# joshuacwnewton/swiftwatcher

Hardware: AMD Instinct MI355X
Metric: frames/sec (segment+classify) on 1080p ROI batches (higher is better)
Workload: dtype f64 (image_filtering), f32 (CNN)

## Files before the change

### include/swk.h

```cpp
#ifndef SWK_H
#define SWK_H

#include <stdint.h>

#ifdef __cplusplus
extern "C" {
#endif

#define SWK_ABI_VERSION 2

enum {
    SWK_OK = 0,
    SWK_ERR_ARG = -1,
    SWK_ERR_HIP = -2,
    SWK_ERR_NOGPU = -3,
    SWK_ERR_CAPACITY = -4,
    SWK_ERR_NOMEM = -5,
    SWK_ERR_STALE = -6
};

enum { SWK_MEM_HOST = 0, SWK_MEM_DEVICE = 1 };

enum { SWK_ORDER_RASTER = 0, SWK_ORDER_BLOCK2X2 = 1 };

// ... 102 lines not shown
                           const swk_segment *segs, const int32_t *nseg, int32_t seg_cap, int32_t min_h, int32_t min_w,
                           const float mean[3], const float std_[3], int32_t pad, int32_t channels_last, int32_t first,
                           int32_t net_cap, float *net, int32_t *seg_frame, int32_t *total, int32_t *skipped);
int32_t swk_segment_inputs_last(swk_ctx *ctx, int32_t min_h, int32_t min_w, const float mean[3], const float std_[3],
                                int32_t pad, int32_t channels_last, int32_t first, int32_t net_cap, float *net,
                                int32_t *seg_frame, int32_t *total, int32_t *skipped);

int32_t swk_nhwc_bias_relu_place(void *stream, const float *src, int32_t n, int32_t sh, int32_t sw, int32_t c, int32_t crop_y,
                                 int32_t crop_x, int32_t h, int32_t w, const float *bias, float *dst, int32_t dH, int32_t dW,
                                 int32_t dC, int32_t off_y, int32_t off_x, int32_t c_off);
int32_t swk_nhwc_maxpool3s2(void *stream, const float *src, int32_t n, int32_t h, int32_t w, int32_t c, float *dst);
int32_t swk_nhwc_head2_relu_mean(void *stream, const float *x, int32_t n, int32_t px, int32_t c, const float *w, const float *bias,
                                 const float *ring, float n_pos, float *out);
int32_t swk_nhwc_conv7x7s2_bias_relu(void *stream, const float *src, int32_t n, int32_t side, int32_t lo, int32_t m, const float *weight,
                                     const float *bias, int32_t cout, float *dst);
int32_t swk_nhwc_conv1x1_bias_relu_place(void *stream, const float *src, int32_t n, int32_t sh, int32_t sw, int32_t cin, int32_t crop_y,
                                         int32_t crop_x, int32_t h, int32_t w, const float *weight, const float *bias, int32_t cout,
                                         float *dst, int32_t dH, int32_t dW, int32_t dC, int32_t off_y, int32_t off_x, int32_t c_off);

int32_t swk_nhwc_maxpool3s2_conv1x1_bias_relu_place(void *stream, const float *src, int32_t n, int32_t t, int32_t cin, const float *weight,
                                                    const float *bias, int32_t cout, float *dst, int32_t dH, int32_t dW, int32_t dC,
                                                    int32_t off_y, int32_t off_x, const float *ring, int32_t live_lo, int32_t live_n);


int32_t swk_nhwc_conv3x3_bias_relu_place(void *stream, const float *src, int32_t n, int32_t t, int32_t cin, const float *weight_t,
                                         const float *bias, int32_t cout, float *dst, int32_t dH, int32_t dW, int32_t dC, int32_t off_y,
                                         int32_t off_x, int32_t c_off);

int32_t swk_winograd_f2x2_3x3_weights(const float *weight, int32_t cout, int32_t cin, float *out);
int32_t swk_nhwc_conv3x3_winograd_bias_relu_place(void *stream, const float *src, int32_t n, int32_t t, int32_t cin, const float *weight_w,
                                                  const float *bias, int32_t cout, float *dst, int32_t dH, int32_t dW, int32_t dC,
                                                  int32_t off_y, int32_t off_x, int32_t c_off);

int32_t swk_track_costs(const double *prev_c, const double *prev_hist0, const uint8_t *prev_has_hist,
                        const double *curr_c, int32_t n_prev, int32_t n_curr, double *cost);
int32_t swk_lsap(const double *cost, int32_t n_rows, int32_t n_cols, int32_t *col4row);

int32_t swk_median_blur_u8(const uint8_t *src, int32_t H, int32_t W, int32_t channels, int32_t ksize, uint8_t *dst);
int32_t swk_otsu_threshold_u8(const uint8_t *src, int64_t count, uint8_t *dst, int32_t *thresh);
int32_t swk_canny_u8(const uint8_t *src, int32_t H, int32_t W, int32_t low, int32_t high, uint8_t *dst);
int32_t swk_dilate_up_u8(const uint8_t *src, int32_t H, int32_t W, int32_t N, uint8_t *dst);
int32_t swk_roi_mask(const uint8_t *frame, int32_t H, int32_t W, int64_t row_stride, const int32_t corners[4],
                     int32_t crop_region[4], uint8_t *mask, int64_t mask_capacity);


#ifdef __cplusplus
}
#endif
#endif
```

### swiftwatcher_amd/_lib.py

```python
import ctypes
import os
import threading

import numpy as np

_HERE = os.path.dirname(os.path.abspath(__file__))
LIB_PATH = os.environ.get("SWK_LIB", os.path.join(_HERE, "libswk.so"))

ABI_VERSION = 2
MEM_HOST, MEM_DEVICE = 0, 1
ERR_STALE = -6
STAGES = ("gray", "rpca", "bilateral", "thresh", "opened", "labels")
ORDER_RASTER, ORDER_BLOCK2X2 = 0, 1
GRAY_Q14, GRAY_Q15 = 0, 1
K_GRAY, K_IALM_STATS, K_IALM_PASS, K_IALM_SMALL, K_FILTER, K_CCL, K_PROPS, K_COPY = range(8)
KERNEL_FAMILIES = ["gray", "ialm_stats", "ialm_pass", "ialm_small", "filter", "ccl", "props", "copy"]

c_u8p = ctypes.POINTER(ctypes.c_uint8)
c_f64p = ctypes.POINTER(ctypes.c_double)
c_i32p = ctypes.POINTER(ctypes.c_int32)


class SwkError(RuntimeError):
    pass
# ... 52 lines not shown
    "swk_batch_run": (ctypes.c_int32, [ctypes.c_void_p, ctypes.POINTER(Input), ctypes.POINTER(Params), ctypes.POINTER(Output)]),
    "swk_batch_run_groups": (ctypes.c_int32, [ctypes.c_void_p, ctypes.POINTER(Input), ctypes.c_int32, ctypes.POINTER(Params), ctypes.POINTER(Output)]),
    "swk_bgr2gray": (ctypes.c_int32, [ctypes.c_void_p, ctypes.c_void_p, ctypes.c_int32, ctypes.c_int32, ctypes.c_int32, ctypes.c_int32, ctypes.c_void_p]),
    "swk_ialm": (ctypes.c_int32, [ctypes.c_void_p, ctypes.c_void_p, ctypes.c_int32, ctypes.c_int32, ctypes.c_double, ctypes.c_double, ctypes.c_int32, ctypes.c_void_p, ctypes.c_void_p, ctypes.c_void_p]),
    "swk_rpca_epilogue": (ctypes.c_int32, [ctypes.c_void_p, ctypes.c_void_p, ctypes.c_int64, ctypes.c_void_p]),
    "swk_bilateral_u8": (ctypes.c_int32, [ctypes.c_void_p, ctypes.c_void_p, ctypes.c_int32, ctypes.c_int32, ctypes.c_int32, ctypes.c_int32, ctypes.c_double, ctypes.c_double, ctypes.c_int32, ctypes.c_void_p]),
    "swk_thresh_tozero_u8": (ctypes.c_int32, [ctypes.c_void_p, ctypes.c_void_p, ctypes.c_int64, ctypes.c_int32, ctypes.c_void_p]),
    "swk_grey_open3x3_u8": (ctypes.c_int32, [ctypes.c_void_p, ctypes.c_void_p, ctypes.c_int32, ctypes.c_int32, ctypes.c_int32, ctypes.c_void_p]),
    "swk_grey_open_u8": (ctypes.c_int32, [ctypes.c_void_p, ctypes.c_void_p] + [ctypes.c_int32] * 5 + [ctypes.c_void_p]),
    "swk_resize_linear_u8": (ctypes.c_int32, [ctypes.c_void_p, ctypes.c_void_p] + [ctypes.c_int32] * 6 + [ctypes.c_void_p]),
    "swk_ccl_u8": (ctypes.c_int32, [ctypes.c_void_p, ctypes.c_void_p, ctypes.c_int32, ctypes.c_int32, ctypes.c_int32, ctypes.c_int32, ctypes.c_int32, ctypes.c_void_p, ctypes.c_void_p]),
    "swk_regionprops_u8": (ctypes.c_int32, [ctypes.c_void_p, ctypes.c_void_p, ctypes.c_int32, ctypes.c_int32, ctypes.c_int32, ctypes.c_int32, ctypes.c_void_p, ctypes.c_void_p]),
    "swk_classifier_input": (ctypes.c_int32, [ctypes.c_void_p, ctypes.c_void_p, ctypes.c_int64, ctypes.c_void_p, ctypes.c_void_p, ctypes.c_int32, ctypes.c_void_p, ctypes.c_void_p, ctypes.c_void_p, ctypes.c_void_p, ctypes.c_int32]),
    "swk_set_sparse_speculation": (ctypes.c_int32, [ctypes.c_void_p, ctypes.c_double]),
    "swk_set_integer_start": (ctypes.c_int32, [ctypes.c_void_p, ctypes.c_int32]),
    "swk_last_integer_start_windows": (ctypes.c_int32, [ctypes.c_void_p, ctypes.c_void_p]),
    "swk_last_eig_sweeps": (ctypes.c_int32, [ctypes.c_void_p, ctypes.c_void_p]),
    "swk_set_norm_speculation": (ctypes.c_int32, [ctypes.c_void_p, ctypes.c_double]),
    "swk_set_norm_guard": (ctypes.c_int32, [ctypes.c_void_p, ctypes.c_double]),
    "swk_prof_guard_windows": (ctypes.c_int32, [ctypes.c_void_p, ctypes.c_void_p]),
    "swk_last_stopping_norms": (ctypes.c_int32, [ctypes.c_void_p, ctypes.c_void_p, ctypes.c_void_p, ctypes.c_int32]),
    "swk_set_start_refine": (ctypes.c_int32, [ctypes.c_void_p, ctypes.c_double]),
    "swk_prof_refined_windows": (ctypes.c_int32, [ctypes.c_void_p, ctypes.c_void_p, ctypes.c_void_p]),
    "swk_prof_pass_bytes_per_element": (ctypes.c_int32, [ctypes.c_void_p, ctypes.c_void_p]),
    "swk_prof_redo_batches": (ctypes.c_int32, [ctypes.c_void_p, ctypes.c_void_p]),
    "swk_prof_redo_windows": (ctypes.c_int32, [ctypes.c_void_p, ctypes.c_void_p]),
    "swk_nhwc_bias_relu_place": (ctypes.c_int32, [ctypes.c_void_p, ctypes.c_void_p] + [ctypes.c_int32] * 8 + [ctypes.c_void_p, ctypes.c_void_p] + [ctypes.c_int32] * 6),
    "swk_set_cnn_tuning": (ctypes.c_int32, [ctypes.c_int32, ctypes.c_int32]),
    "swk_nhwc_conv7x7s2_bias_relu": (ctypes.c_int32, [ctypes.c_void_p, ctypes.c_void_p, ctypes.c_int32, ctypes.c_int32, ctypes.c_int32, ctypes.c_int32, ctypes.c_void_p, ctypes.c_void_p, ctypes.c_int32, ctypes.c_void_p]),
    "swk_nhwc_conv1x1_bias_relu_place": (ctypes.c_int32, [ctypes.c_void_p, ctypes.c_void_p] + [ctypes.c_int32] * 8 + [ctypes.c_void_p, ctypes.c_void_p, ctypes.c_int32, ctypes.c_void_p] + [ctypes.c_int32] * 6),
    "swk_nhwc_conv3x3_bias_relu_place": (ctypes.c_int32, [ctypes.c_void_p, ctypes.c_void_p, ctypes.c_int32, ctypes.c_int32, ctypes.c_int32, ctypes.c_void_p, ctypes.c_void_p, ctypes.c_int32, ctypes.c_void_p] + [ctypes.c_int32] * 6),
    "swk_nhwc_conv3x3_winograd_bias_relu_place": (ctypes.c_int32, [ctypes.c_void_p, ctypes.c_void_p, ctypes.c_int32, ctypes.c_int32, ctypes.c_int32, ctypes.c_void_p, ctypes.c_void_p, ctypes.c_int32, ctypes.c_void_p] + [ctypes.c_int32] * 6),
    "swk_winograd_f2x2_3x3_weights": (ctypes.c_int32, [ctypes.c_void_p, ctypes.c_int32, ctypes.c_int32, ctypes.c_void_p]),
    "swk_nhwc_maxpool3s2_conv1x1_bias_relu_place": (ctypes.c_int32, [ctypes.c_void_p, ctypes.c_void_p, ctypes.c_int32, ctypes.c_int32, ctypes.c_int32, ctypes.c_void_p, ctypes.c_void_p, ctypes.c_int32, ctypes.c_void_p] + [ctypes.c_int32] * 5 + [ctypes.c_void_p, ctypes.c_int32, ctypes.c_int32]),
    "swk_nhwc_maxpool3s2": (ctypes.c_int32, [ctypes.c_void_p, ctypes.c_void_p, ctypes.c_int32, ctypes.c_int32, ctypes.c_int32, ctypes.c_int32, ctypes.c_void_p]),
    "swk_nhwc_head2_relu_mean": (ctypes.c_int32, [ctypes.c_void_p, ctypes.c_void_p, ctypes.c_int32, ctypes.c_int32, ctypes.c_int32, ctypes.c_void_p,
                                                  ctypes.c_void_p, ctypes.c_void_p, ctypes.c_float, ctypes.c_void_p]),
    "swk_segment_inputs": (ctypes.c_int32, [ctypes.c_void_p, ctypes.c_void_p, ctypes.c_int32, ctypes.c_int32, ctypes.c_void_p, ctypes.c_void_p, ctypes.c_int32, ctypes.c_int32, ctypes.c_int32, ctypes.c_void_p, ctypes.c_void_p, ctypes.c_int32, ctypes.c_int32, ctypes.c_int32, ctypes.c_int32, ctypes.c_void_p, ctypes.c_void_p, ctypes.c_void_p, ctypes.c_void_p]),
    "swk_segment_inputs_last": (ctypes.c_int32, [ctypes.c_void_p, ctypes.c_int32, ctypes.c_int32, ctypes.c_void_p, ctypes.c_void_p, ctypes.c_int32, ctypes.c_int32, ctypes.c_int32, ctypes.c_int32, ctypes.c_void_p, ctypes.c_void_p, ctypes.c_void_p, ctypes.c_void_p]),
    "swk_device_alloc": (ctypes.c_int32, [ctypes.c_void_p, ctypes.c_int64, ctypes.POINTER(ctypes.c_void_p)]),
    "swk_device_free": (ctypes.c_int32, [ctypes.c_void_p, ctypes.c_void_p]),
    "swk_device_read": (ctypes.c_int32, [ctypes.c_void_p, ctypes.c_void_p, ctypes.c_void_p, ctypes.c_int64]),
    "swk_classifier_input_window": (ctypes.c_int32, [ctypes.c_void_p, ctypes.c_void_p, ctypes.c_int64, ctypes.c_void_p, ctypes.c_void_p, ctypes.c_int32, ctypes.c_void_p, ctypes.c_void_p, ctypes.c_int32, ctypes.c_int32, ctypes.c_void_p, ctypes.c_void_p, ctypes.c_int32]),
    "swk_track_costs": (ctypes.c_int32, [ctypes.c_void_p, ctypes.c_void_p, ctypes.c_void_p, ctypes.c_void_p, ctypes.c_int32, ctypes.c_int32, ctypes.c_void_p]),
    "swk_lsap": (ctypes.c_int32, [ctypes.c_void_p, ctypes.c_int32, ctypes.c_int32, ctypes.c_void_p]),
    "swk_median_blur_u8": (ctypes.c_int32, [ctypes.c_void_p, ctypes.c_int32, ctypes.c_int32, ctypes.c_int32, ctypes.c_int32, ctypes.c_void_p]),
    "swk_otsu_threshold_u8": (ctypes.c_int32, [ctypes.c_void_p, ctypes.c_int64, ctypes.c_void_p, ctypes.c_void_p]),
    "swk_canny_u8": (ctypes.c_int32, [ctypes.c_void_p, ctypes.c_int32, ctypes.c_int32, ctypes.c_int32, ctypes.c_int32, ctypes.c_void_p]),
    "swk_dilate_up_u8": (ctypes.c_int32, [ctypes.c_void_p, ctypes.c_int32, ctypes.c_int32, ctypes.c_int32, ctypes.c_void_p]),
    "swk_roi_mask": (ctypes.c_int32, [ctypes.c_void_p, ctypes.c_int32, ctypes.c_int32, ctypes.c_int64, ctypes.c_void_p, ctypes.c_void_p, ctypes.c_void_p, ctypes.c_int64]),
    "swk_pinned_alloc": (ctypes.c_int32, [ctypes.c_int32, ctypes.c_int64, ctypes.POINTER(ctypes.c_void_p)]),
    "swk_pinned_free": (ctypes.c_int32, [ctypes.c_void_p]),
    "swk_cut_boxes": (ctypes.c_int32, [ctypes.c_void_p, ctypes.c_int32, ctypes.c_int64, ctypes.c_int32, ctypes.c_int32, ctypes.c_void_p, ctypes.c_void_p, ctypes.c_void_p, ctypes.c_void_p]),
    "swk_stage_frames": (ctypes.c_int32, [ctypes.c_void_p, ctypes.c_int32, ctypes.c_int64, ctypes.c_int32, ctypes.c_int32, ctypes.c_int64, ctypes.c_int64, ctypes.c_void_p, ctypes.c_int32]),
    "swk_prof_enable": (ctypes.c_int32, [ctypes.c_void_p, ctypes.c_int32]),
    "swk_prof_reset": (ctypes.c_int32, [ctypes.c_void_p]),
    "swk_prof_get": (ctypes.c_int32, [ctypes.c_void_p, ctypes.c_int32, ctypes.POINTER(ctypes.c_double), ctypes.POINTER(ctypes.c_int64)]),
    "swk_prof_window_iters": (ctypes.c_int32, [ctypes.c_void_p, ctypes.POINTER(ctypes.c_int64)]),
    "swk_set_ialm_variant": (ctypes.c_int32, [ctypes.c_void_p, ctypes.c_int32]),
    "swk_set_pass_tuning": (ctypes.c_int32, [ctypes.c_void_p, ctypes.c_int32]),
    "swk_set_eig_method": (ctypes.c_int32, [ctypes.c_void_p, ctypes.c_int32]),
}
EXPORTS = sorted(_SIGS)


def _preload_torch_hip_runtime():
# ... 630 lines not shown
```

### swiftwatcher_amd/csrc/build.py

```python
import os
import subprocess
import sys

HERE = os.path.dirname(os.path.abspath(__file__))
PKG = os.path.dirname(HERE)
ROOT = os.path.dirname(PKG)
LIB = os.path.join(PKG, "libswk.so")
SOURCES = ["swk_api.hip", "ialm.hip", "ialm_mfma.hip", "ialm_mstate.hip", "ialm_small.hip", "ialm_refine.hip", "ialm_gram8.hip", "groups.hip", "filters.hip", "ccl.hip", "classify_input.hip", "cnn_aux.hip", "cnn_conv1.hip", "cnn_conv1x1.hip", "cnn_expand_bf16.hip", "cnn_conv3x3.hip", "cnn_wino3x3.hip", "cnn_poolsq.hip", "tracker.cpp", "roi_mask.cpp", "host_stage.cpp"]
HEADERS = ["swk_internal.h", "ialm_small_dev.h", os.path.join(ROOT, "include", "swk.h"), os.path.join(ROOT, "include", "swk_debug.h")]
FLAGS = ["--offload-arch=gfx950", "-O3", "-std=c++17", "-fPIC", "-ffp-contract=off",
         "-fvisibility=hidden", "-Wall", "-Wno-unused-function", "-I", os.path.join(ROOT, "include"), "-I", HERE]


def _stale(out, deps):
    if not os.path.exists(out):
        return True
    t = os.path.getmtime(out)
    return any(os.path.getmtime(d) > t for d in deps)


def build(force=False, verbose=False):
    hipcc = os.environ.get("HIPCC", "/opt/rocm/bin/hipcc")
    objdir = os.path.join(HERE, "build")
    os.makedirs(objdir, exist_ok=True)
    hdrs = [h if os.path.isabs(h) else os.path.join(HERE, h) for h in HEADERS]
    objs = []
    procs = []
    for src in SOURCES:
        sp = os.path.join(HERE, src)
        obj = os.path.join(objdir, src + ".o")
        objs.append(obj)
        if force or _stale(obj, [sp] + hdrs + [os.path.abspath(__file__)]):
            cmd = [hipcc] + FLAGS + ["-c", sp, "-o", obj]
            if verbose:
                print(" ".join(cmd))
            procs.append((src, subprocess.Popen(cmd)))
    for src, p in procs:
        if p.wait() != 0:
            raise RuntimeError("hipcc failed on " + src)
    if force or procs or _stale(LIB, objs):
        cmd = [hipcc, "--offload-arch=gfx950", "-shared", "-fPIC", "-pthread", "-o", LIB] + objs
# ... 9 lines not shown
```

### swiftwatcher_amd/segment_classification.py

```python
import ctypes
import os
import threading

import numpy as np
import torch
from torch import nn

IMAGENET_MEAN = (0.485, 0.456, 0.406)
IMAGENET_STD = (0.229, 0.224, 0.225)
RESIZE = 24
PAD = (224 - 24) // 2


class Fire(nn.Module):

    def __init__(self, inplanes, squeeze_planes, expand1x1_planes, expand3x3_planes):
        super().__init__()
        self.squeeze = nn.Conv2d(inplanes, squeeze_planes, kernel_size=1)
        self.squeeze_activation = nn.ReLU(inplace=True)
        self.expand1x1 = nn.Conv2d(squeeze_planes, expand1x1_planes, kernel_size=1)
        self.expand1x1_activation = nn.ReLU(inplace=True)
        self.expand3x3 = nn.Conv2d(squeeze_planes, expand3x3_planes, kernel_size=3, padding=1)
        self.expand3x3_activation = nn.ReLU(inplace=True)

# ... 74 lines not shown
                lo, hi = a, b
            else:
                out_size = maps[i + 1].shape[-1] if i + 1 < len(feats) else x.shape[-1]
                a, b = _affected(lo, hi, 3, 2, 0, out_size)
                n0, n1 = 2 * a, 2 * b + 2
                assert n0 >= 0 and n1 <= size - 1
                tile = in_map[:, :, n0:n1 + 1, n0:n1 + 1].contiguous()
                self.plan.append(("pool", layer, tile, lo - n0, hi - lo + 1, None, None))
                lo, hi, size = a, b, out_size
        self.final = (lo, hi, size)
        self.final_bg = x[:, :, lo:hi + 1, lo:hi + 1].contiguous()
        ring = head.clone()
        ring[:, :, lo:hi + 1, lo:hi + 1] = 0
        self.ring_sum = ring.sum(dim=(2, 3))
        self.n_pos = float(size * size)
        self.sq_bg = []
        with torch.no_grad():
            for kind, layer, tile, off, n, pad, crop in self.plan:
                if kind != "fire":
                    self.sq_bg.append(None)
                    continue
                sq = layer.squeeze_activation(layer.squeeze(tile))
                if pad[0] or pad[1]:
                    sq = torch.nn.functional.pad(sq, (pad[0], pad[1], pad[0], pad[1]))
                self.sq_bg.append(sq.contiguous())
        self._cap = 0
        self._buf = None
        self.memory_format = torch.channels_last if dev.type == "cuda" else torch.contiguous_format
        if self.memory_format == torch.channels_last:
            model.to(memory_format=torch.channels_last)
        self.own_kernels = os.environ.get("SWK_OWN_CNN_KERNELS", "1") == "1"
        self._head = None
        self.winograd = True
        self.fuse_pool = os.environ.get("SWK_FUSE_POOL", "1") == "1"
        self._w1 = None
        self._wt3 = {}
        self._ww3 = {}

    def macs_per_segment(self):
        m = self.model
        c1 = m.features[0]
        side = (self.IN_HI - self.IN_LO + 1 - 7) // 2 + 1
        executed = useful = side * side * c1.out_channels * c1.in_channels * 49
        last_n = None
        on_gpu = self.ring_sum.is_cuda and self.memory_format == torch.channels_last and self.own_kernels
        for kind, layer, tile, off, n, pad, crop in self.plan:
            if kind != "fire":
                continue
            t = tile.shape[2] + pad[0] + pad[1]
            sq, e1, e3 = layer.squeeze, layer.expand1x1, layer.expand3x3
            executed += n * n * sq.out_channels * sq.in_channels
            e1_side = n if on_gpu else t
            executed += e1_side * e1_side * e1.out_channels * e1.in_channels
            wino = on_gpu and self.winograd and e3.out_channels == 4 * e3.in_channels and e3.in_channels in (16, 32, 48, 64)
            if wino:
                tiles = ((t - 2 + 1) // 2) ** 2
                executed += tiles * 16 * e3.out_channels * e3.in_channels
            else:
                executed += (t - 2) ** 2 * e3.out_channels * e3.in_channels * 9
            useful += n * n * sq.out_channels * sq.in_channels
            useful += crop[1] ** 2 * (e1.out_channels * e1.in_channels + e3.out_channels * e3.in_channels * 9)
            last_n = crop[1]
        head = m.classifier[1]
        executed += last_n * last_n * head.out_channels * head.in_channels
        useful += last_n * last_n * head.out_channels * head.in_channels
        return int(executed), int(useful)

    def _buffers(self, batch):
        if batch <= self._cap:
            return self._buf
        bufs = []
        for (kind, layer, tile, off, n, pad, crop), sq in zip(self.plan, self.sq_bg):
            if kind == "fire":
                bufs.append(sq.expand(batch, -1, -1, -1).contiguous(memory_format=self.memory_format))
            else:
                bufs.append(tile.expand(batch, -1, -1, -1).contiguous(memory_format=self.memory_format))
        live = []
        for j, (kind, layer, tile, off, n, pad, crop) in enumerate(self.plan):
            nxt = self.plan[j + 1][0] if j + 1 < len(self.plan) else "head"
            if kind == "fire" and nxt != "pool":
                if nxt == "fire":
                    _, _, ntile, noff, nn, _, _ = self.plan[j + 1]
                    bg = ntile[:, :, noff:noff + nn, noff:noff + nn]
                else:
                    bg = self.final_bg
                assert bg.shape[2] == crop[1] and bg.shape[1] == layer.expand1x1.out_channels + layer.expand3x3.out_channels
                live.append(bg.expand(batch, -1, -1, -1).contiguous(memory_format=self.memory_format))
            else:
                live.append(None)
        self._buf, self._cap = (bufs, live), batch
        self.version = getattr(self, "version", 0) + 1
        return self._buf

    def _gpu_path(self, tiles):
        return tiles.is_cuda and self.memory_format == torch.channels_last and all(
            kind != "fire" or not (pad[0] or pad[1]) for kind, _, _, _, _, pad, _ in self.plan)

    def reserve(self, batch):
        self._buffers(batch)
        if self.ring_sum.is_cuda:
            self._aux_buffers(batch)

    @torch.no_grad()
    def __call__(self, tiles, row0=0):
        if self._gpu_path(tiles):
            with torch.cuda.device(tiles.device):
                return self._forward_hip_glue(tiles, row0)
        if row0:
            raise ValueError("row0 is a feature of the GPU path")
        m = self.model
        conv2d = torch.nn.functional.conv2d
        k = tiles.shape[0]
        bufs, live = self._buffers(k)
        x = torch.relu(m.features[0](tiles.contiguous(memory_format=self.memory_format)))
        a, b = self.pool1_slice
        x = m.features[2](x[:, :, a:b, a:b])
        for j, (kind, layer, tile, off, n, pad, crop) in enumerate(self.plan):
            if kind == "pool":
                x = layer(bufs[j][:k])
                continue
            sq = bufs[j][:k]
            o = off + pad[0]
            torch.clamp_min(layer.squeeze(x), 0, out=sq[:, :, o:o + n, o:o + n])
            e3 = conv2d(sq, layer.expand3x3.weight, layer.expand3x3.bias)
            e1 = conv2d(sq, layer.expand1x1.weight, layer.expand1x1.bias)
            c, cn = crop
            c1 = layer.expand1x1.out_channels
            if live[j] is not None:
                dest = live[j][:k]
            else:
                _, _, _, poff, pn, _, _ = self.plan[j + 1]
                assert pn == cn
                dest = bufs[j + 1][:k, :, poff:poff + pn, poff:poff + pn]
            cp = c + pad[0]
# ... 7 lines not shown
        from . import _lib
        lib = _lib.load()
        stream = ctypes.c_void_p(torch.cuda.current_stream(tiles.device).cuda_stream)
        m = self.model
        conv2d = torch.nn.functional.conv2d
        k = tiles.shape[0]
        bufs, live = self._buffers(row0 + k)
        rows = slice(row0, row0 + k)
        cl = torch.channels_last

        def nhwc(t):
            return t if t.is_contiguous(memory_format=cl) else t.contiguous(memory_format=cl)

        def place(e, bias, dest, crop, size, off, c_off):
            e = nhwc(e)
            rc = lib.swk_nhwc_bias_relu_place(stream, e.data_ptr(), k, e.shape[2], e.shape[3], e.shape[1], crop, crop, size, size,
                                              bias.data_ptr(), dest.data_ptr(), dest.shape[2], dest.shape[3], dest.shape[1],
                                              off, off, c_off)
            if rc:
                raise RuntimeError("swk_nhwc_bias_relu_place failed (%d)" % rc)

        def conv1x1(src, crop, size, conv, dest, off, c_off):
            src = nhwc(src)
            wgt = conv.weight.reshape(conv.out_channels, conv.in_channels)
            rc = lib.swk_nhwc_conv1x1_bias_relu_place(stream, src.data_ptr(), k, src.shape[2], src.shape[3], src.shape[1], crop, crop,
                                                      size, size, wgt.data_ptr(), conv.bias.data_ptr(), conv.out_channels,
                                                      dest.data_ptr(), dest.shape[2], dest.shape[3], dest.shape[1], off, off, c_off)
            if rc:
                raise RuntimeError("swk_nhwc_conv1x1_bias_relu_place failed (%d)" % rc)

        def conv3x3(src, j, conv, dest, off, c_off):
            src = nhwc(src)
            cin, cout = conv.in_channels, conv.out_channels
            if self.winograd and cout == 4 * cin and cin in (16, 32, 48, 64) and k * src.shape[2] * src.shape[2] * cin * 4 < (1 << 32):
                ww = self._ww3.get(j)
                if ww is None:
                    w = conv.weight.detach().to("cpu", torch.float32).contiguous()
                    out = torch.empty(16 * cin * cout, dtype=torch.float32)
                    if lib.swk_winograd_f2x2_3x3_weights(w.data_ptr(), cout, cin, out.data_ptr()):
                        raise RuntimeError("swk_winograd_f2x2_3x3_weights failed")
                    ww = self._ww3[j] = out.to(src.device)
                rc = lib.swk_nhwc_conv3x3_winograd_bias_relu_place(stream, src.data_ptr(), k, src.shape[2], cin, ww.data_ptr(),
                                                                   conv.bias.data_ptr(), cout, dest.data_ptr(), dest.shape[2],
                                                                   dest.shape[3], dest.shape[1], off, off, c_off)
                if rc:
                    raise RuntimeError("swk_nhwc_conv3x3_winograd_bias_relu_place failed (%d)" % rc)
                return
            wt = self._wt3.get(j)
            if wt is None:
                wt = self._wt3[j] = conv.weight.detach().permute(2, 3, 1, 0).contiguous(memory_format=torch.contiguous_format)
            assert src.shape[2] == src.shape[3]
            rc = lib.swk_nhwc_conv3x3_bias_relu_place(stream, src.data_ptr(), k, src.shape[2], src.shape[1], wt.data_ptr(),
                                                      conv.bias.data_ptr(), conv.out_channels, dest.data_ptr(), dest.shape[2],
                                                      dest.shape[3], dest.shape[1], off, off, c_off)
            if rc:
                raise RuntimeError("swk_nhwc_conv3x3_bias_relu_place failed (%d)" % rc)

        def pool(src, dst):
            rc = lib.swk_nhwc_maxpool3s2(stream, src.data_ptr(), k, src.shape[2], src.shape[3], src.shape[1], dst.data_ptr())
            if rc:
                raise RuntimeError("swk_nhwc_maxpool3s2 failed (%d)" % rc)

        def pool_squeeze(src, conv, dest, off, ring=None, live=(0, 0)):
            wgt = conv.weight.reshape(conv.out_channels, conv.in_channels)
            rc = lib.swk_nhwc_maxpool3s2_conv1x1_bias_relu_place(stream, src.data_ptr(), k, src.shape[2], src.shape[1], wgt.data_ptr(),
                                                                 conv.bias.data_ptr(), conv.out_channels, dest.data_ptr(), dest.shape[2],
                                                                 dest.shape[3], dest.shape[1], off, off,
                                                                 None if ring is None else ring.data_ptr(), live[0], live[1])
            if rc:
                raise RuntimeError("swk_nhwc_maxpool3s2_conv1x1_bias_relu_place failed (%d)" % rc)

        aux = self._aux_buffers(row0 + k)
        conv1 = m.features[0]
        a, b = self.pool1_slice
        c1buf = aux["conv1"][rows]
        side = tiles.shape[2]
        if self.own_kernels and conv1.out_channels == 96 and side % 2 == 0 and 2 * (b - 1) + 8 <= side:
            if self._w1 is None:
                self._w1 = conv1.weight.detach().contiguous(memory_format=torch.contiguous_format).clone()
            xin = nhwc(tiles)
            rc = lib.swk_nhwc_conv7x7s2_bias_relu(stream, xin.data_ptr(), k, side, a, b - a, self._w1.data_ptr(), conv1.bias.data_ptr(),
                                                  conv1.out_channels, c1buf.data_ptr())
            if rc:
                raise RuntimeError("swk_nhwc_conv7x7s2_bias_relu failed (%d)" % rc)
        else:
            e = conv2d(nhwc(tiles), conv1.weight, None, stride=conv1.stride)
            place(e, conv1.bias, c1buf, a, b - a, 0, 0)
        fuse = self.fuse_pool and self.own_kernels
        to_pool = c1buf
        pool_ring, pool_live = None, (0, 0)
        x = aux["pool_in"][rows]
        if not fuse:
            pool(c1buf, x)
        pi = 0
        for j, (kind, layer, tile, off, n, pad, crop) in enumerate(self.plan):
            if kind == "pool":
                x = aux["pool_out"][pi][rows]
                if fuse:
                    to_pool, pool_ring, pool_live = bufs[j][rows], bufs[j][0:1], (off, n)
                else:
                    pool(bufs[j][rows], x)
                pi += 1
                continue
            sq = bufs[j][rows]
            c, cn = crop
            c1 = layer.expand1x1.out_channels
            if live[j] is not None:
                dest, doff = live[j][rows], 0
            else:
                dest, doff = bufs[j + 1][rows], self.plan[j + 1][3]
            if self.own_kernels:
                if fuse and to_pool is not None:
                    assert (to_pool.shape[2] - 3) // 2 + 1 == n
                    pool_squeeze(to_pool, layer.squeeze, sq, off, pool_ring, pool_live)
                    to_pool = None
                else:
                    conv1x1(x, 0, n, layer.squeeze, sq, off, 0)
                conv1x1(sq, off, n, layer.expand1x1, dest, doff + off - c, 0)
            else:
                place(conv2d(x, layer.squeeze.weight, None), layer.squeeze.bias, sq, 0, n, off, 0)
                e1 = conv2d(sq, layer.expand1x1.weight, None)
                place(e1, layer.expand1x1.bias, dest, c, cn, doff, 0)
            if self.own_kernels:
                conv3x3(sq, j, layer.expand3x3, dest, doff, c1)
            else:
                place(conv2d(sq, layer.expand3x3.weight, None), layer.expand3x3.bias, dest, 0, cn, doff, c1)
            x = dest
        head = m.classifier[1]
        if self.own_kernels and head.out_channels == 2 and x.shape[1] in (256, 512, 768, 1024) and x.is_contiguous(memory_format=cl):
            if self._head is None:
                self._head = (head.weight.detach().reshape(2, -1).contiguous(), head.bias.detach().contiguous(),
                              self.ring_sum.reshape(-1).contiguous())
            hw, hb, ring = self._head
            out = torch.empty((k, 2), dtype=torch.float32, device=x.device)
            rc = lib.swk_nhwc_head2_relu_mean(stream, x.data_ptr(), k, x.shape[2] * x.shape[3], x.shape[1], hw.data_ptr(), hb.data_ptr(),
                                              ring.data_ptr(), self.n_pos, out.data_ptr())
            if rc:
                raise RuntimeError("swk_nhwc_head2_relu_mean failed (%d)" % rc)
            return out
        px = x.permute(0, 2, 3, 1).reshape(-1, x.shape[1])
        s = torch.relu(torch.nn.functional.linear(px, head.weight.view(head.out_channels, -1), head.bias))
        s = s.view(k, -1, head.out_channels).sum(dim=1)
        return (s + self.ring_sum) / self.n_pos

    def _aux_buffers(self, batch):
        if getattr(self, "_aux_cap", 0) >= batch:
            return self._aux
        dev = self.ring_sum.device
        cl = torch.channels_last

        def buf(c, h):
            return torch.empty((batch, c, h, h), dtype=torch.float32, device=dev).contiguous(memory_format=cl)

        a, b = self.pool1_slice
        conv1_c = self.model.features[0].out_channels
        aux = {"conv1": buf(conv1_c, b - a), "pool_in": buf(conv1_c, (b - a - 3) // 2 + 1), "pool_out": []}
        for kind, layer, tile, off, n, pad, crop in self.plan:
            if kind == "pool":
                aux["pool_out"].append(buf(tile.shape[1], (tile.shape[2] - 3) // 2 + 1))
        self._aux, self._aux_cap = aux, batch
        self.version = getattr(self, "version", 0) + 1
        return aux


def setup_model(num_classes):
    model = SqueezeNet10(num_classes)
# ... 267 lines not shown
```

Measured before the change: 39570.

## Add split-bf16 MFMA Winograd 3x3 expand conv kernel with operand prewarming

```diff
diff --git a/include/swk.h b/include/swk.h
--- a/include/swk.h
+++ b/include/swk.h
@@ -158,6 +158,11 @@
                                                   const float *bias, int32_t cout, float *dst, int32_t dH, int32_t dW, int32_t dC,
                                                   int32_t off_y, int32_t off_x, int32_t c_off);
 
+int32_t swk_winograd_f2x2_3x3_weights_bf16s(const float *weight, int32_t cout, int32_t cin, uint16_t *out);
+int32_t swk_nhwc_conv3x3_winograd_bf16s_bias_relu_place(void *stream, const float *src, int32_t n, int32_t t, int32_t cin,
+                                                        const uint16_t *weight_s, const float *bias, int32_t cout, float *dst, int32_t dH,
+                                                        int32_t dW, int32_t dC, int32_t off_y, int32_t off_x, int32_t c_off);
+
 int32_t swk_track_costs(const double *prev_c, const double *prev_hist0, const uint8_t *prev_has_hist,
                         const double *curr_c, int32_t n_prev, int32_t n_curr, double *cost);
 int32_t swk_lsap(const double *cost, int32_t n_rows, int32_t n_cols, int32_t *col4row);
diff --git a/swiftwatcher_amd/_lib.py b/swiftwatcher_amd/_lib.py
--- a/swiftwatcher_amd/_lib.py
+++ b/swiftwatcher_amd/_lib.py
@@ -108,6 +108,8 @@
     "swk_nhwc_conv3x3_bias_relu_place": (ctypes.c_int32, [ctypes.c_void_p, ctypes.c_void_p, ctypes.c_int32, ctypes.c_int32, ctypes.c_int32, ctypes.c_void_p, ctypes.c_void_p, ctypes.c_int32, ctypes.c_void_p] + [ctypes.c_int32] * 6),
     "swk_nhwc_conv3x3_winograd_bias_relu_place": (ctypes.c_int32, [ctypes.c_void_p, ctypes.c_void_p, ctypes.c_int32, ctypes.c_int32, ctypes.c_int32, ctypes.c_void_p, ctypes.c_void_p, ctypes.c_int32, ctypes.c_void_p] + [ctypes.c_int32] * 6),
     "swk_winograd_f2x2_3x3_weights": (ctypes.c_int32, [ctypes.c_void_p, ctypes.c_int32, ctypes.c_int32, ctypes.c_void_p]),
+    "swk_nhwc_conv3x3_winograd_bf16s_bias_relu_place": (ctypes.c_int32, [ctypes.c_void_p, ctypes.c_void_p, ctypes.c_int32, ctypes.c_int32, ctypes.c_int32, ctypes.c_void_p, ctypes.c_void_p, ctypes.c_int32, ctypes.c_void_p] + [ctypes.c_int32] * 6),
+    "swk_winograd_f2x2_3x3_weights_bf16s": (ctypes.c_int32, [ctypes.c_void_p, ctypes.c_int32, ctypes.c_int32, ctypes.c_void_p]),
     "swk_nhwc_maxpool3s2_conv1x1_bias_relu_place": (ctypes.c_int32, [ctypes.c_void_p, ctypes.c_void_p, ctypes.c_int32, ctypes.c_int32, ctypes.c_int32, ctypes.c_void_p, ctypes.c_void_p, ctypes.c_int32, ctypes.c_void_p] + [ctypes.c_int32] * 5 + [ctypes.c_void_p, ctypes.c_int32, ctypes.c_int32]),
     "swk_nhwc_maxpool3s2": (ctypes.c_int32, [ctypes.c_void_p, ctypes.c_void_p, ctypes.c_int32, ctypes.c_int32, ctypes.c_int32, ctypes.c_int32, ctypes.c_void_p]),
     "swk_nhwc_head2_relu_mean": (ctypes.c_int32, [ctypes.c_void_p, ctypes.c_void_p, ctypes.c_int32, ctypes.c_int32, ctypes.c_int32, ctypes.c_void_p,
diff --git a/swiftwatcher_amd/csrc/build.py b/swiftwatcher_amd/csrc/build.py
--- a/swiftwatcher_amd/csrc/build.py
+++ b/swiftwatcher_amd/csrc/build.py
@@ -6,7 +6,7 @@
 PKG = os.path.dirname(HERE)
 ROOT = os.path.dirname(PKG)
 LIB = os.path.join(PKG, "libswk.so")
-SOURCES = ["swk_api.hip", "ialm.hip", "ialm_mfma.hip", "ialm_mstate.hip", "ialm_small.hip", "ialm_refine.hip", "ialm_gram8.hip", "groups.hip", "filters.hip", "ccl.hip", "classify_input.hip", "cnn_aux.hip", "cnn_conv1.hip", "cnn_conv1x1.hip", "cnn_expand_bf16.hip", "cnn_conv3x3.hip", "cnn_wino3x3.hip", "cnn_poolsq.hip", "tracker.cpp", "roi_mask.cpp", "host_stage.cpp"]
+SOURCES = ["swk_api.hip", "ialm.hip", "ialm_mfma.hip", "ialm_mstate.hip", "ialm_small.hip", "ialm_refine.hip", "ialm_gram8.hip", "groups.hip", "filters.hip", "ccl.hip", "classify_input.hip", "cnn_aux.hip", "cnn_conv1.hip", "cnn_conv1x1.hip", "cnn_expand_bf16.hip", "cnn_conv3x3.hip", "cnn_wino3x3.hip", "cnn_wino3x3_bf16s.hip", "cnn_poolsq.hip", "tracker.cpp", "roi_mask.cpp", "host_stage.cpp"]
 HEADERS = ["swk_internal.h", "ialm_small_dev.h", os.path.join(ROOT, "include", "swk.h"), os.path.join(ROOT, "include", "swk_debug.h")]
 FLAGS = ["--offload-arch=gfx950", "-O3", "-std=c++17", "-fPIC", "-ffp-contract=off",
          "-fvisibility=hidden", "-Wall", "-Wno-unused-function", "-I", os.path.join(ROOT, "include"), "-I", HERE]
diff --git a/swiftwatcher_amd/csrc/cnn_wino3x3_bf16s.hip b/swiftwatcher_amd/csrc/cnn_wino3x3_bf16s.hip
--- /dev/null
+++ b/swiftwatcher_amd/csrc/cnn_wino3x3_bf16s.hip
@@ -0,0 +1,303 @@
+#include "swk_internal.h"
+
+#include <cstring>
+
+namespace swk {
+
+typedef float f16v __attribute__((ext_vector_type(16)));
+typedef __bf16 bf16x8 __attribute__((ext_vector_type(8)));
+
+static int wino_bf16s_spp(int cin, int cout) { return cin == 64 && cout == 256 ? 2 : cin / 16; }
+
+template <int KG> struct WinoVPad { static constexpr int value = KG == 6 ? 3 : 16 / KG; };
+
+template <int NBLK, int SPP>
+__global__ __launch_bounds__(64 * NBLK, 2) void k_wino3x3_bf16s_relu_place(const float *__restrict__ src, int nseg, int t, int T,
+                                                                          const uint16_t *__restrict__ wu, const float *__restrict__ bias,
+                                                                          int cout, float *__restrict__ dst, int dH, int dW, int dC, int off_y,
+                                                                          int off_x, int c_off, FastDiv fTT, FastDiv fT)
+{
+    constexpr int NW = NBLK, NT = 64 * NW, KG = NBLK, CIN = 8 * KG, S = CIN / 16, PHS = S / SPP, SLOTS = 64, NP = 32 * NBLK;
+    constexpr int VT = SLOTS + WinoVPad<KG>::value;
+    constexpr int WPB = SPP * 3 * 1024;
+    static_assert(S % SPP == 0 && NT == SLOTS * KG, "one staging item per thread");
+    extern __shared__ uint4 lds_w[];
+    char *const Wl = (char *)lds_w;
+    uint4 *const V0 = (uint4 *)(Wl + 2 * NW * WPB), *const V1 = V0 + 3 * KG * VT;
+    float *const lbias = (float *)(V1 + 3 * KG * VT);
+    const int tid = threadIdx.x, lane = tid & 63, wave = tid >> 6, r = lane & 31, hh = lane >> 5;
+    const int o = t - 2, TT = T * T;
+    const int64_t ntiles = (int64_t)nseg * TT, src_floats = (int64_t)nseg * t * t * CIN;
+    const int64_t ntasks = (ntiles + SLOTS - 1) / SLOTS;
+    for (int i = tid; i < NP; i += NT) lbias[i] = i < cout ? bias[i] : 0.0f;
+
+    const int sg = tid % KG, sslot = tid / KG;
+    unsigned sbase;
+    int slim;
+    const char *const srcb = (const char *)src;
+    auto stage_setup = [&](int64_t task) {
+        int64_t m = task * SLOTS + sslot;
+        if (m >= ntiles) m = ntiles - 1;
+        const unsigned bu = fTT.div((unsigned)m), rem = (unsigned)m - bu * (unsigned)TT, ty = fT.div(rem), tx = rem - ty * (unsigned)T;
+        const int64_t b = bu;
+        const int64_t base = (((b * t + 2 * ty) * t + 2 * tx) * (int64_t)CIN + 8 * sg) * 4;
+        const int64_t lim = src_floats * 4 - 32 - base;
+        sbase = (unsigned)base;
+        slim = (int)(lim < (1 << 30) ? lim : (1 << 30));
+    };
+    float4 st[4][2];
+    auto stage_issue = [&](int p) {
+        const int xi = p >> 2, nu = p & 3;
+        const int ra0 = (0x1210 >> (4 * xi)) & 15, ra1 = (0x3122 >> (4 * xi)) & 15;
+        const int rb0 = (0x1210 >> (4 * nu)) & 15, rb1 = (0x3122 >> (4 * nu)) & 15;
+        const int os[4] = {(ra0 * t + rb0) * (CIN * 4), (ra0 * t + rb1) * (CIN * 4), (ra1 * t + rb0) * (CIN * 4), (ra1 * t + rb1) * (CIN * 4)};
+#pragma unroll
+        for (int i = 0; i < 4; ++i) {
+            const char *q = srcb + (sbase + (unsigned)(os[i] < slim ? os[i] : slim));
+            st[i][0] = *(const float4 *)q;
+            st[i][1] = *(const float4 *)(q + 16);
+        }
+    };
+    auto stage_store = [&](int p, uint4 *Vn) {
+        const float sx = (p >> 2) == 1 ? 1.0f : -1.0f, sn = (p & 3) == 1 ? 1.0f : -1.0f;
+        bf16x8 v1, v2, v3;
+#pragma unroll
+        for (int h = 0; h < 2; ++h) {
+            const float a[4] = {st[0][h].x, st[0][h].y, st[0][h].z, st[0][h].w}, b[4] = {st[1][h].x, st[1][h].y, st[1][h].z, st[1][h].w},
+                        c[4] = {st[2][h].x, st[2][h].y, st[2][h].z, st[2][h].w}, d[4] = {st[3][h].x, st[3][h].y, st[3][h].z, st[3][h].w};
+#pragma unroll
+            for (int e = 0; e < 4; ++e) {
+                const float v = __builtin_fmaf(__builtin_fmaf(d[e], sn, c[e]), sx, __builtin_fmaf(b[e], sn, a[e]));
+                const __bf16 x1 = (__bf16)v;
+                const float r1 = v - (float)x1;
+                const __bf16 x2 = (__bf16)r1;
+                v1[4 * h + e] = x1; v2[4 * h + e] = x2; v3[4 * h + e] = (__bf16)(r1 - (float)x2);
+            }
+        }
+        uint4 *q = Vn + sg * VT + sslot;
+        q[0] = __builtin_bit_cast(uint4, v1);
+        q[KG * VT] = __builtin_bit_cast(uint4, v2);
+        q[2 * KG * VT] = __builtin_bit_cast(uint4, v3);
+    };
+
+    const unsigned wvoff = (unsigned)(lane * 16);
+    auto w_issue = [&](int g, int buf) {
+        const char *gp = (const char *)wu + ((int64_t)g * NW + __builtin_amdgcn_readfirstlane(wave)) * WPB;
+        const unsigned l = __builtin_amdgcn_readfirstlane((unsigned)(uintptr_t)(Wl + (buf * NW + wave) * WPB));
+#pragma unroll
+        for (int sub = 0; sub < SPP; ++sub) {
+            unsigned keep;
+            asm volatile("s_mov_b32 %0, m0\n\ts_mov_b32 m0, %2\n\ts_nop 0\n\tglobal_load_lds_dwordx4 %1, %3\n\t"
+                         "global_load_lds_dwordx4 %1, %3 offset:1024\n\tglobal_load_lds_dwordx4 %1, %3 offset:2048\n\ts_mov_b32 m0, %0"
+                         : "=&s"(keep) : "v"(wvoff), "s"(l + sub * 3072u), "s"(gp + sub * 3072) : "memory");
+        }
+    };
+    auto wait_copies = [&]() { asm volatile("s_waitcnt vmcnt(0)" ::: "memory"); };
+    auto wait_copies_keep8 = [&]() { asm volatile("s_waitcnt vmcnt(8)" ::: "memory"); };
+
+    int64_t task = blockIdx.x;
+    if (task < ntasks) {
+        stage_setup(task);
+        stage_issue(0);
+        stage_store(0, V0);
+        w_issue(0, 0);
+    }
+    wait_copies();
+    __syncthreads();
+    for (; task < ntasks; task += gridDim.x) {
+        int64_t ro[2];
+        bool valid[2], vy1[2], vx1[2];
+#pragma unroll
+        for (int tg = 0; tg < 2; ++tg) {
+            const int64_t m = task * SLOTS + tg * 32 + r;
+            valid[tg] = m < ntiles;
+            const int64_t mm = valid[tg] ? m : ntiles - 1;
+            const unsigned bu = fTT.div((unsigned)mm), rem = (unsigned)mm - bu * (unsigned)TT;
+            const int ty = (int)fT.div(rem), tx = (int)(rem - (unsigned)ty * (unsigned)T);
+            const int64_t b = bu;
+            ro[tg] = ((b * dH + off_y + 2 * ty) * dW + off_x + 2 * tx) * (int64_t)dC + c_off + 32 * wave + 4 * hh;
+            vy1[tg] = 2 * ty + 1 < o;
+            vx1[tg] = 2 * tx + 1 < o;
+        }
+        const bool more = task + gridDim.x < ntasks;
+        f16v Y[2][2][2];
+#pragma unroll
+        for (int i = 0; i < 2; ++i)
+#pragma unroll
+            for (int j = 0; j < 2; ++j)
+#pragma unroll
+                for (int tg = 0; tg < 2; ++tg)
+#pragma unroll
+                    for (int e = 0; e < 16; ++e) Y[i][j][tg][e] = 0.0f;
+        auto phase = [&](const char *Wb, const uint4 *Vc, int s0, f16v *M) {
+            const uint4 *wq = (const uint4 *)Wb + lane;
+#pragma unroll
+            for (int sub = 0; sub < SPP; ++sub) {
+                const int s = s0 + sub;
+                const bf16x8 u1 = __builtin_bit_cast(bf16x8, wq[(3 * sub) * 64]), u2 = __builtin_bit_cast(bf16x8, wq[(3 * sub + 1) * 64]),
+                             u3 = __builtin_bit_cast(bf16x8, wq[(3 * sub + 2) * 64]);
+#pragma unroll
+                for (int tg = 0; tg < 2; ++tg) {
+                    const uint4 *vq = Vc + (2 * s + hh) * VT + 32 * tg + r;
+                    const bf16x8 x1 = __builtin_bit_cast(bf16x8, vq[0]), x2 = __builtin_bit_cast(bf16x8, vq[KG * VT]),
+                                 x3 = __builtin_bit_cast(bf16x8, vq[2 * KG * VT]);
+                    M[tg] = __builtin_amdgcn_mfma_f32_32x32x16_bf16(u1, x3, M[tg], 0, 0, 0);
+                    M[tg] = __builtin_amdgcn_mfma_f32_32x32x16_bf16(u2, x2, M[tg], 0, 0, 0);
+                    M[tg] = __builtin_amdgcn_mfma_f32_32x32x16_bf16(u3, x1, M[tg], 0, 0, 0);
+                    M[tg] = __builtin_amdgcn_mfma_f32_32x32x16_bf16(u1, x2, M[tg], 0, 0, 0);
+                    M[tg] = __builtin_amdgcn_mfma_f32_32x32x16_bf16(u2, x1, M[tg], 0, 0, 0);
+                    M[tg] = __builtin_amdgcn_mfma_f32_32x32x16_bf16(u1, x1, M[tg], 0, 0, 0);
+                }
+            }
+        };
+        for (int p = 0; p < 16; ++p) {
+            const uint4 *Vc = (p & 1) ? V1 : V0;
+            uint4 *Vn = (p & 1) ? V0 : V1;
+            const int pn = (p + 1) & 15;
+            if (p == 15 && more) stage_setup(task + gridDim.x);
+            const int xi = p >> 2, nu = p & 3;
+            const float ax[2] = {xi < 3 ? 1.0f : 0.0f, xi == 0 ? 0.0f : xi == 1 ? 1.0f : -1.0f};
+            const float an[2] = {nu < 3 ? 1.0f : 0.0f, nu == 0 ? 0.0f : nu == 1 ? 1.0f : -1.0f};
+            f16v M[2];
+#pragma unroll
+            for (int tg = 0; tg < 2; ++tg)
+#pragma unroll
+                for (int e = 0; e < 16; ++e) M[tg][e] = 0.0f;
+#pragma unroll
+            for (int h = 0; h < PHS; ++h) {
+                const int g = p * PHS + h, gn = g + 1 == 16 * PHS ? 0 : g + 1;
+                w_issue(gn, (g + 1) & 1);
+                if (h == 0) stage_issue(pn);
+                phase(Wl + ((g & 1) * NW + wave) * WPB, Vc, h * SPP, M);
+                if (h == PHS - 1) {
+                    stage_store(pn, Vn);
+#pragma unroll
+                    for (int i = 0; i < 2; ++i)
+#pragma unroll
+                        for (int j = 0; j < 2; ++j) {
+                            const float c = ax[i] * an[j];
+                            if (c != 0.0f) {
+#pragma unroll
+                                for (int tg = 0; tg < 2; ++tg)
+#pragma unroll
+                                    for (int e = 0; e < 16; ++e) Y[i][j][tg][e] = __builtin_fmaf(M[tg][e], c, Y[i][j][tg][e]);
+                            }
+                        }
+                }
+                if (h == 0 && PHS > 1) wait_copies_keep8();
+                else wait_copies();
+                if (h == PHS - 1) __syncthreads();
+            }
+        }
+#pragma unroll
+        for (int tg = 0; tg < 2; ++tg) {
+            if (!valid[tg]) continue;
+#pragma unroll
+            for (int i = 0; i < 2; ++i)
+#pragma unroll
+                for (int j = 0; j < 2; ++j) {
+                    if ((i == 1 && !vy1[tg]) || (j == 1 && !vx1[tg])) continue;
+                    float *q = dst + ro[tg] + ((int64_t)i * dW + j) * dC;
+#pragma unroll
+                    for (int gq = 0; gq < 4; ++gq) {
+                        const int c = 32 * wave + 8 * gq + 4 * hh;
+                        if (c < cout) {
+                            const float4 b4 = *(const float4 *)(lbias + c);
+                            float4 v;
+                            v.x = fmaxf(Y[i][j][tg][4 * gq] + b4.x, 0.0f);
+                            v.y = fmaxf(Y[i][j][tg][4 * gq + 1] + b4.y, 0.0f);
+                            v.z = fmaxf(Y[i][j][tg][4 * gq + 2] + b4.z, 0.0f);
+                            v.w = fmaxf(Y[i][j][tg][4 * gq + 3] + b4.w, 0.0f);
+                            *(float4 *)(q + 8 * gq) = v;
+                        }
+                    }
+                }
+        }
+    }
+}
+
+template <int NBLK, int SPP>
+static int launch_wino3x3_bf16s(hipStream_t s, const float *src, int n, int t, const uint16_t *wu, const float *bias, int cout, float *dst,
+                                int dH, int dW, int dC, int off_y, int off_x, int c_off)
+{
+    constexpr int NW = NBLK, KG = NBLK, CIN = 8 * NBLK, VT = 64 + WinoVPad<KG>::value;
+    const size_t lds = (size_t)2 * NW * SPP * 3 * 1024 + (size_t)2 * 3 * KG * VT * 16 + 32 * NBLK * sizeof(float);
+    static_assert((size_t)2 * NW * SPP * 3 * 1024 + (size_t)2 * 3 * KG * VT * 16 + 32 * NBLK * 4 <= 160 * 1024 - 256, "LDS of one workgroup");
+    static unsigned long long attr_mask = 0;
+    if (!ensure_dyn_lds((const void *)k_wino3x3_bf16s_relu_place<NBLK, SPP>, 160 * 1024 - 256, attr_mask)) return SWK_ERR_HIP;
+    if ((int64_t)n * t * t * CIN * 4 >= ((int64_t)1 << 32)) return SWK_ERR_CAPACITY;
+    const int T = (t - 2 + 1) / 2;
+    const int64_t ntiles = (int64_t)n * T * T;
+    int64_t blocks = (ntiles + 63) / 64;
+    const int64_t by_lds = (int64_t)((160 * 1024 - 256) / lds), by_waves = 8 / NW;
+    const int64_t per_cu = by_waves < 1 ? 1 : (by_lds < by_waves ? by_lds : by_waves);
+    if (blocks > 256 * per_cu) blocks = 256 * per_cu;
+    hipLaunchKernelGGL((k_wino3x3_bf16s_relu_place<NBLK, SPP>), dim3((unsigned)blocks), dim3(64 * NW), lds, s, src, n, t, T, wu, bias, cout, dst,
+                       dH, dW, dC, off_y, off_x, c_off, FastDiv((unsigned)(T * T)), FastDiv((unsigned)T));
+    return hipGetLastError() == hipSuccess ? SWK_OK : SWK_ERR_HIP;
+}
+
+}
+
+#pragma GCC visibility push(default)
+extern "C" {
+
+int32_t swk_winograd_f2x2_3x3_weights_bf16s(const float *weight, int32_t cout, int32_t cin, uint16_t *out)
+{
+    if (!weight || !out || cout < 1 || cin < 16 || (cin & 15)) return SWK_ERR_ARG;
+    const int spp = swk::wino_bf16s_spp(cin, cout), S = cin / 16, PHS = S / spp, CG = (cout + 31) / 32;
+    if (S % spp) return SWK_ERR_ARG;
+    static const double G[4][3] = {{1.0, 0.0, 0.0}, {0.5, 0.5, 0.5}, {0.5, -0.5, 0.5}, {0.0, 0.0, 1.0}};
+    for (int64_t i = 0, e = (int64_t)16 * cin * CG * 32 * 3; i < e; ++i) out[i] = 0;
+    auto bf16_rne = [](float f, float &back) -> uint16_t {
+        uint32_t u;
+        memcpy(&u, &f, 4);
+        u = (u + 0x7fffu + ((u >> 16) & 1u)) & 0xffff0000u;
+        memcpy(&back, &u, 4);
+        return (uint16_t)(u >> 16);
+    };
+    for (int co = 0; co < cout; ++co)
+        for (int ci = 0; ci < cin; ++ci) {
+            const float *g = weight + ((int64_t)co * cin + ci) * 9;
+            double tmp[4][3], U[4][4];
+            for (int a = 0; a < 4; ++a)
+                for (int c = 0; c < 3; ++c) tmp[a][c] = G[a][0] * g[c] + G[a][1] * g[3 + c] + G[a][2] * g[6 + c];
+            for (int a = 0; a < 4; ++a)
+                for (int c = 0; c < 4; ++c) U[a][c] = tmp[a][0] * G[c][0] + tmp[a][1] * G[c][1] + tmp[a][2] * G[c][2];
+            const int s = ci >> 4, ph = s / spp, sub = s % spp, lane = ((ci >> 3) & 1) * 32 + (co & 31), j = ci & 7, cb = co >> 5;
+            for (int p = 0; p < 16; ++p) {
+                const float u = (float)U[p >> 2][p & 3];
+                float b1, b2, b3;
+                const uint16_t h1 = bf16_rne(u, b1);
+                const float r1 = u - b1;
+                const uint16_t h2 = bf16_rne(r1, b2);
+                const uint16_t h3 = bf16_rne(r1 - b2, b3);
+                const int64_t blk = (((int64_t)p * PHS + ph) * CG + cb) * spp + sub;
+                out[((blk * 3 + 0) * 64 + lane) * 8 + j] = h1;
+                out[((blk * 3 + 1) * 64 + lane) * 8 + j] = h2;
+                out[((blk * 3 + 2) * 64 + lane) * 8 + j] = h3;
+            }
+        }
+    return SWK_OK;
+}
+
+int32_t swk_nhwc_conv3x3_winograd_bf16s_bias_relu_place(void *stream, const float *src, int32_t n, int32_t t, int32_t cin,
+                                                        const uint16_t *weight_s, const float *bias, int32_t cout, float *dst, int32_t dH,
+                                                        int32_t dW, int32_t dC, int32_t off_y, int32_t off_x, int32_t c_off)
+{
+    if (!src || !weight_s || !bias || !dst || n < 1 || t < 3 || cout < 4 || (cout & 3) || (dC & 3) || (c_off & 3) || off_y < 0 || off_x < 0 ||
+        off_y + t - 2 > dH || off_x + t - 2 > dW || c_off < 0 || c_off + cout > dC || (((uintptr_t)src | (uintptr_t)dst | (uintptr_t)weight_s) & 15))
+        return SWK_ERR_ARG;
+    using namespace swk;
+    hipStream_t s = (hipStream_t)stream;
+#define SWK_W3S_ARGS s, src, n, t, weight_s, bias, cout, dst, dH, dW, dC, off_y, off_x, c_off
+    if (cin == 16 && cout == 64) return launch_wino3x3_bf16s<2, 1>(SWK_W3S_ARGS);
+    if (cin == 32 && cout == 128) return launch_wino3x3_bf16s<4, 2>(SWK_W3S_ARGS);
+    if (cin == 48 && cout == 192) return launch_wino3x3_bf16s<6, 3>(SWK_W3S_ARGS);
+    if (cin == 64 && cout == 256) return launch_wino3x3_bf16s<8, 2>(SWK_W3S_ARGS);
+#undef SWK_W3S_ARGS
+    return SWK_ERR_ARG;
+}
+
+}
+#pragma GCC visibility pop
diff --git a/swiftwatcher_amd/segment_classification.py b/swiftwatcher_amd/segment_classification.py
--- a/swiftwatcher_amd/segment_classification.py
+++ b/swiftwatcher_amd/segment_classification.py
@@ -130,10 +130,12 @@
         self.own_kernels = os.environ.get("SWK_OWN_CNN_KERNELS", "1") == "1"
         self._head = None
         self.winograd = True
+        self.wino_split_bf16 = os.environ.get("SWK_WINO_SPLIT_BF16", "1") == "1"
         self.fuse_pool = os.environ.get("SWK_FUSE_POOL", "1") == "1"
         self._w1 = None
         self._wt3 = {}
         self._ww3 = {}
+        self._ws3 = {}
 
     def macs_per_segment(self):
         m = self.model
@@ -198,6 +200,61 @@
         self._buffers(batch)
         if self.ring_sum.is_cuda:
             self._aux_buffers(batch)
+            self._prepare_operands()
+
+    def _prepare_operands(self):
+        if not (self.own_kernels and self.ring_sum.is_cuda and self.memory_format == torch.channels_last):
+            return
+        self._conv1_operand()
+        for j, (kind, layer, tile, off, n, pad, crop) in enumerate(self.plan):
+            if kind == "fire":
+                self._w3_operand(j, layer.expand3x3)
+        self._head_operand()
+
+    def _conv1_operand(self):
+        if self._w1 is None:
+            self._w1 = self.model.features[0].weight.detach().contiguous(memory_format=torch.contiguous_format).clone()
+        return self._w1
+
+    def _head_operand(self):
+        if self._head is None:
+            head = self.model.classifier[1]
+            self._head = (head.weight.detach().reshape(head.out_channels, -1).contiguous(), head.bias.detach().contiguous(),
+                          self.ring_sum.reshape(-1).contiguous())
+        return self._head
+
+    def _w3_kind(self, conv):
+        cin, cout = conv.in_channels, conv.out_channels
+        if self.winograd and cout == 4 * cin and cin in (16, 32, 48, 64):
+            return "bf16s" if self.wino_split_bf16 and cin != 16 else "f32"
+        return "direct"
+
+    def _w3_operand(self, j, conv, kind=None):
+        from . import _lib
+        kind = kind or self._w3_kind(conv)
+        cache = {"bf16s": self._ws3, "f32": self._ww3, "direct": self._wt3}[kind]
+        w = cache.get(j)
+        if w is not None:
+            return w
+        cin, cout = conv.in_channels, conv.out_channels
+        dev = conv.weight.device
+        if kind == "direct":
+            w = conv.weight.detach().permute(2, 3, 1, 0).contiguous(memory_format=torch.contiguous_format)
+        else:
+            lib = _lib.load()
+            wc = conv.weight.detach().to("cpu", torch.float32).contiguous()
+            ncol = 32 * (-(-cout // 32))
+            if kind == "bf16s":
+                out = torch.empty(3 * 16 * cin * ncol, dtype=torch.int16)
+                if lib.swk_winograd_f2x2_3x3_weights_bf16s(wc.data_ptr(), cout, cin, out.data_ptr()):
+                    raise RuntimeError("swk_winograd_f2x2_3x3_weights_bf16s failed")
+            else:
+                out = torch.empty(16 * cin * ncol, dtype=torch.float32)
+                if lib.swk_winograd_f2x2_3x3_weights(wc.data_ptr(), cout, cin, out.data_ptr()):
+                    raise RuntimeError("swk_winograd_f2x2_3x3_weights failed")
+            w = out.to(dev)
+        cache[j] = w
+        return w
 
     @torch.no_grad()
     def __call__(self, tiles, row0=0):
@@ -271,23 +328,16 @@
         def conv3x3(src, j, conv, dest, off, c_off):
             src = nhwc(src)
             cin, cout = conv.in_channels, conv.out_channels
-            if self.winograd and cout == 4 * cin and cin in (16, 32, 48, 64) and k * src.shape[2] * src.shape[2] * cin * 4 < (1 << 32):
-                ww = self._ww3.get(j)
-                if ww is None:
-                    w = conv.weight.detach().to("cpu", torch.float32).contiguous()
-                    out = torch.empty(16 * cin * cout, dtype=torch.float32)
-                    if lib.swk_winograd_f2x2_3x3_weights(w.data_ptr(), cout, cin, out.data_ptr()):
-                        raise RuntimeError("swk_winograd_f2x2_3x3_weights failed")
-                    ww = self._ww3[j] = out.to(src.device)
-                rc = lib.swk_nhwc_conv3x3_winograd_bias_relu_place(stream, src.data_ptr(), k, src.shape[2], cin, ww.data_ptr(),
-                                                                   conv.bias.data_ptr(), cout, dest.data_ptr(), dest.shape[2],
-                                                                   dest.shape[3], dest.shape[1], off, off, c_off)
+            kind = self._w3_kind(conv)
+            if kind != "direct" and k * src.shape[2] * src.shape[2] * cin * 4 < (1 << 32):
+                ww = self._w3_operand(j, conv, kind)
+                fn = "swk_nhwc_conv3x3_winograd_bf16s_bias_relu_place" if kind == "bf16s" else "swk_nhwc_conv3x3_winograd_bias_relu_place"
+                rc = getattr(lib, fn)(stream, src.data_ptr(), k, src.shape[2], cin, ww.data_ptr(), conv.bias.data_ptr(), cout,
+                                      dest.data_ptr(), dest.shape[2], dest.shape[3], dest.shape[1], off, off, c_off)
                 if rc:
-                    raise RuntimeError("swk_nhwc_conv3x3_winograd_bias_relu_place failed (%d)" % rc)
+                    raise RuntimeError("%s failed (%d)" % (fn, rc))
                 return
-            wt = self._wt3.get(j)
-            if wt is None:
-                wt = self._wt3[j] = conv.weight.detach().permute(2, 3, 1, 0).contiguous(memory_format=torch.contiguous_format)
+            wt = self._w3_operand(j, conv, "direct")
             assert src.shape[2] == src.shape[3]
             rc = lib.swk_nhwc_conv3x3_bias_relu_place(stream, src.data_ptr(), k, src.shape[2], src.shape[1], wt.data_ptr(),
                                                       conv.bias.data_ptr(), conv.out_channels, dest.data_ptr(), dest.shape[2],
@@ -315,10 +365,9 @@
         c1buf = aux["conv1"][rows]
         side = tiles.shape[2]
         if self.own_kernels and conv1.out_channels == 96 and side % 2 == 0 and 2 * (b - 1) + 8 <= side:
-            if self._w1 is None:
-                self._w1 = conv1.weight.detach().contiguous(memory_format=torch.contiguous_format).clone()
+            w1 = self._conv1_operand()
             xin = nhwc(tiles)
-            rc = lib.swk_nhwc_conv7x7s2_bias_relu(stream, xin.data_ptr(), k, side, a, b - a, self._w1.data_ptr(), conv1.bias.data_ptr(),
+            rc = lib.swk_nhwc_conv7x7s2_bias_relu(stream, xin.data_ptr(), k, side, a, b - a, w1.data_ptr(), conv1.bias.data_ptr(),
                                                   conv1.out_channels, c1buf.data_ptr())
             if rc:
                 raise RuntimeError("swk_nhwc_conv7x7s2_bias_relu failed (%d)" % rc)
@@ -367,10 +416,7 @@
             x = dest
         head = m.classifier[1]
         if self.own_kernels and head.out_channels == 2 and x.shape[1] in (256, 512, 768, 1024) and x.is_contiguous(memory_format=cl):
-            if self._head is None:
-                self._head = (head.weight.detach().reshape(2, -1).contiguous(), head.bias.detach().contiguous(),
-                              self.ring_sum.reshape(-1).contiguous())
-            hw, hb, ring = self._head
+            hw, hb, ring = self._head_operand()
             out = torch.empty((k, 2), dtype=torch.float32, device=x.device)
             rc = lib.swk_nhwc_head2_relu_mean(stream, x.data_ptr(), k, x.shape[2] * x.shape[3], x.shape[1], hw.data_ptr(), hb.data_ptr(),
                                               ring.data_ptr(), self.n_pos, out.data_ptr())
```

Result: faster. 42220 (median of 6 runs) (+6.7%).
